# neilcouture/halo2-svd041

Measured on AMD Instinct MI355X. Metric: advice cells/sec (SVD-verify witness gen, N×N) at 1/2/4/8 MI355X, higher is better.
Workload: dtype bn254_fr (u32 limbs; exact multi-modular int8 MFMA GEMM); 1 GPU; svd_verify_witness N=1024 M=1024 PRECISION_BITS=63 LOOKUP_BITS=19, one matrix per GPU; N=1024, M=1024, precision_bits=63, lookup_bits=19, parallelism=replicas x1 (no data-path collective), ranks=1

## Files before the change

### halo2_svd041_amd/csrc/engine.cpp

```cpp
#include <math.h>
#include <stdio.h>
#include <stdlib.h>
#include <string.h>

#include <algorithm>

#include "engine_internal.hpp"
#include "ingest.hpp"
#include "ingest_dev.hpp"
#include "export.hpp"
#include "commit.hpp"

struct BigU {
    Fr v;
};
static BigU big_from_words(const uint64_t w[4]) { return BigU{fr_raw_words(w)}; }
static BigU big_from_u128(unsigned __int128 x) {
    BigU b;
    b.v = fr_zero();
    for (int i = 0; i < 4; ++i) b.v.w[i] = (uint32_t)(x >> (32 * i));
    return b;
}
static int big_bits(const BigU& b) {
    for (int i = 7; i >= 0; --i)
// ... 605 lines not shown
        shard_rows(c, R, &r0, &r1);
        if (R > 1) {
            eb = (uint32_t)(r0 * cw);
            ee = (uint32_t)(r1 * cw);
        }
    }
    if (g_stage_log) {
        uint32_t nmul = 0;
        for (uint32_t i = 0; i < a.nmo; ++i) nmul += a.mo[i].op == MO_MUL;
        const int sid = c->st == c->st_cell ? 1 : c->st == c->st2 ? 2 : c->st == c->st3 ? 3 : 0;
        fprintf(stderr, "stage %-28s elems %8u C %3u L %3u nv %2u nmo %2u muls %u nk %u  s%d\n", tag, ee - eb,
                a.C, a.L, a.nv, a.nmo, nmul, a.nk, sid);
        if (getenv("SVDW_STAGE_LOG")[0] == '2') {
            fprintf(stderr, "  slots");
            for (uint32_t k = 0; k < a.C + a.L; ++k) {
                const SlotOp& o = k < a.C ? a.adv[k] : a.lk[k - a.C];
                fprintf(stderr, " %u:%u:%u", o.src, o.lo, o.nbits);
            }
            fprintf(stderr, "\n");
        }
    }
    if (c->dry || ee <= eb) return;
    a.out_adv = cellp(c, phase, off);
    a.out_lk = a.L ? c->ph[phase].lk + loff : nullptr;
    for (int k = 0; k < kMaxViews; ++k) a.view[k] = f64_view(c, a.view[k]);
    a.e_begin = eb;
    a.e_end = ee;
    a.cols = cols ? cols : 1;
    a.flags = c->opt.stage_flags;
    bool heavy = false;
    for (uint32_t i = 0; i < a.nmo; ++i)
        heavy |= a.mo[i].op == MO_MUL || a.mo[i].op == MO_ISZERO || a.mo[i].op == MO_POWK;
    a.E = heavy ? kStageElems : c->opt.stage_elems;
    while (a.E > 64 && stage_lds_bytes(a.nv ? a.nv : 1, a.E, a.C + a.L) > 65536) a.E -= 64;
    auto magic = [](uint64_t d) -> uint32_t { return d > 1 ? (uint32_t)(((1ull << 32) + d - 1) / d) : 0; };
    a.cdiv_magic = magic(a.C);
    a.ldiv_magic = magic(a.L);
    uint32_t loads = 0;
    for (uint32_t i = 0; i < a.nmo; ++i) loads += a.mo[i].op == MO_LOAD;
    const double bytes = 32.0 * (ee - eb) * ((double)a.C + a.L + loads);
    for (auto& b : c->batches) {
        if (b.st != c->st || !stage_multi_fits(a)) continue;
        auto reads = [&](const svdw_ctx::Pending& q) {
            const char* w0 = reinterpret_cast<const char*>(q.a.out_adv);
            const char* w1 = w0 + sizeof(Fr) * (uint64_t)q.a.e_end * q.a.C;
            for (int k = 0; k < kMaxViews; ++k) {
                const DView& v = a.view[k];
                if (!v.ptr || v.mode == VIEW_DIAGK) continue;
                const int64_t dr = (int64_t)(v.rows ? v.rows - 1 : 0) * v.rs,
                              dc = (int64_t)(v.cols ? v.cols - 1 : 0) * v.cs;
                const int64_t lo = std::min<int64_t>(dr, 0) + std::min<int64_t>(dc, 0),
                              hi = std::max<int64_t>(dr, 0) + std::max<int64_t>(dc, 0) + 1;
                const char* p = reinterpret_cast<const char*>(v.ptr);
                if (p + lo * (int64_t)sizeof(Fr) < w1 && p + hi * (int64_t)sizeof(Fr) > w0) return true;
            }
            return false;
        };
        size_t g = 0;
        for (size_t k = 0; k < b.groups.size(); ++k)
            for (const auto& q : b.groups[k])
                if (reads(q)) g = k + 1;
        if (c->call.stage_front && g == 0) {
            b.groups.insert(b.groups.begin(), std::vector<svdw_ctx::Pending>{});
            b.groups[0].push_back({a, std::string("k_stage:") + tag, bytes});
            b.last = 0;
            return;
        }
// ... 1830 lines not shown
};
template <auto Member>
static void set_opt(svdw_ctx* c, int64_t v) {
    c->opt.*Member = static_cast<std::remove_reference_t<decltype(c->opt.*Member)>>(v);
}
static void set_lanes(svdw_ctx* c, int64_t v) { c->lanes = (int)v; }
static void set_pipeline(svdw_ctx* c, int64_t v) {
    c->opt.pipeline = (int)v;
    if (!v) {
        release_alt(c);
        if (c->lane) release_alt(c->lane);
    }
}
static void set_stage_rot(svdw_ctx* c, int64_t v) {
    c->opt.stage_flags = v ? (c->opt.stage_flags | STAGE_ROT) : (c->opt.stage_flags & ~STAGE_ROT);
}
static const char kStageElemsMsg[] = "stage_elems: a multiple of 16 in [16, 256]";
static void set_stage_elems(svdw_ctx* c, int64_t v) {
    REQUIRE(v % 16 == 0, kStageElemsMsg);
    c->opt.stage_elems = (uint32_t)v;
}
static void set_commit_window_bits(svdw_ctx* c, int64_t v) {
    REQUIRE(v != 1, "commit_window_bits: 0 (the plan) or 2..16");
    c->opt.commit_window_bits = (uint32_t)v;
}
using Opt = svdw_ctx::Options;
static const OptionDef kOptions[] = {
    {"lanes", 1, 2, "lanes: 1 or 2", set_lanes},
    {"pipeline", 0, 1, "pipeline: 0 or 1", set_pipeline},
    {"vm_linear", 0, 1, "vm_linear: 0 or 1", set_opt<&Opt::vm_linear>},
    {"graph", 0, 1, "graph: 0 or 1", set_opt<&Opt::graph_vm>},
    {"gemm_impl", SVDW_GEMM_MFMA, SVDW_GEMM_VALU, "gemm_impl: 0 (mfma) or 1 (valu)", set_opt<&Opt::gemm_impl>},
    {"stage_elems", 16, 256, kStageElemsMsg, set_stage_elems},
    {"prod_cell", -1, 1, "prod_cell: -1, 0 or 1", set_opt<&Opt::prod_cell>},
    {"phase1_overlap", 0, 2, "phase1_overlap: 0, 1 or 2", set_opt<&Opt::phase1_overlap>},
    {"hold_us", 0, 100000, "hold_us: 0..100000", set_opt<&Opt::hold_us>},
    {"rlc_prefix", INT64_MIN, INT64_MAX, "", set_opt<&Opt::rlc_prefix>},
    {"res_f64", INT64_MIN, INT64_MAX, "", set_opt<&Opt::res_f64>},
    {"gemm_crt", 0, 1, "gemm_crt: 0 or 1", set_opt<&Opt::gemm_crt>},
    {"res_wait", -1, 1, "res_wait: -1 (auto), 0 or 1", set_opt<&Opt::res_wait>},
    {"place_trials", 0, 8, "place_trials: 0..8", set_opt<&Opt::place_trials>},
    {"stage_rot", 0, 1, "stage_rot: 0 or 1", set_stage_rot},
    {"gemm_kern", -1, 2, "gemm_kern: -1 (auto), 0, 1 or 2", set_opt<&Opt::gemm_kern>},
    {"stage_batch", INT64_MIN, INT64_MAX, "", set_opt<&Opt::stage_batch>},
    {"f64_views", INT64_MIN, INT64_MAX, "", set_opt<&Opt::f64_views>},
    {"p1_at", -1, 3, "p1_at: -1 (auto), 0, 1, 2 or 3", set_opt<&Opt::p1_at>},
    {"commit_window_bits", 0, kCommitMaxBits, "commit_window_bits: 0 (the plan) or 2..16", set_commit_window_bits},
    {"commit_scratch_mib", 1, 65536, "commit_scratch_mib: 1..65536", set_opt<&Opt::commit_scratch_mib>},
    {"dchk_at", 0, 2, "dchk_at: 0 (cell stream), 1 (st2) or 2 (st3)", set_opt<&Opt::dchk_at>},
    {"gamma_at", -1, 1, "gamma_at: -1 (auto), 0 (cell stream) or 1 (st3)", set_opt<&Opt::gamma_at>},
    {"overlap", INT64_MIN, INT64_MAX, "", set_opt<&Opt::overlap>},
};
static_assert(std::is_nothrow_move_constructible<svdw_ctx>::value && std::is_nothrow_move_assignable<svdw_ctx>::value, "svdw_ctx moves");
static void lane_switch(svdw_ctx* c) {
    if (!c->lane) {
        svdw_ctx* L = new svdw_ctx();
        L->P = c->P;
        L->LB = c->LB;
        L->device = c->device;
        L->dry = false;
        try {
            ctx_init_device(L);
        } catch (...) {
            ctx_release(L);
            throw;
        }
// ... 1516 lines not shown
```

### halo2_svd041_amd/csrc/engine_internal.hpp

```cpp
#pragma once
#include <hip/hip_runtime.h>
#include <stdint.h>

#include <array>
#include <chrono>
#include <functional>
#include <new>
#include <set>
#include <stdexcept>
#include <string>
#include <tuple>
#include <vector>

#include "../../include/svdw.h"
#include "kernels.hpp"

using namespace svdw;

inline thread_local std::string g_err;
struct SvdwError {
    int code;
    std::string msg;
};
[[noreturn]] inline void fail(int code, const std::string& msg) { throw SvdwError{code, msg}; }
// ... 38 lines not shown
inline void fr_store_words(const Fr& x, uint64_t w[4]) {
    for (int i = 0; i < 4; ++i) w[i] = (uint64_t)x.w[2 * i] | ((uint64_t)x.w[2 * i + 1] << 32);
}
inline bool fr_reduced(const Fr& x) {
    Fr t;
    return sub_p(t, x) != 0;
}

struct ProverState {
    DBuf scratch;
    std::vector<char> upload;
    std::vector<Fr> omega;
    uint32_t omega_k = 0;
    DBuf ntt_tab, ntt_tmp;
    uint32_t ntt_k = 0;
    DBuf commit_ws;
    DBuf basis, basis_tmp;
    uint32_t basis_k = 0, basis_ek = 0, basis_unusable = 0;
    Fr basis_shift{};
    std::vector<DBuf*> dbufs() { return {&scratch, &ntt_tab, &ntt_tmp, &basis, &basis_tmp, &commit_ws}; }
};

struct Stream {
    Fr* adv = nullptr;
    uint64_t n = 0, cap = 0;
    Fr* lk = nullptr;
    uint64_t nl = 0, lcap = 0;
};
struct svdw_ctx {
    struct Options {
        int gemm_impl = SVDW_GEMM_MFMA;
        uint32_t stage_flags = STAGE_ALIGN | STAGE_ROT;
        uint32_t stage_elems = kStageElems;
        int gemm_crt = 1;
        int gemm_kern = -1;
        int res_wait = -1;
        int place_trials = 6;
        bool res_f64 = true;
        int phase1_overlap = 1;
        int prod_cell = 1;
        uint32_t hold_us = 0;
        uint32_t commit_window_bits = 0;
        uint32_t commit_scratch_mib = 1024;
        bool rlc_prefix = false;
        int p1_at = -1;
        int dchk_at = 0, gamma_at = -1;
        bool f64_views = true;
        bool overlap = true;
        bool stage_batch = true;
        int graph_vm = 1;
        int vm_linear = 1;
        int pipeline = 1;
        uint32_t shard_rank = 0, shard_world = 1;
        bool prof = false;
        std::string prof_filter;
        bool host_trace = false;
        auto tied() const {
            return std::tie(gemm_impl, stage_flags, stage_elems, gemm_crt, gemm_kern, res_wait, place_trials,
                            res_f64, phase1_overlap, prod_cell, hold_us, rlc_prefix, p1_at, dchk_at, gamma_at,
                            f64_views, overlap, stage_batch, graph_vm, vm_linear, pipeline, shard_rank,
                            shard_world, prof, prof_filter, host_trace);
        }
        bool operator==(const Options& o) const { return tied() == o.tied(); }
    } opt;
    struct PreGemm {
        uint64_t off;
        hipEvent_t ev;
        hipStream_t st;
    };
    struct F64Src { svdw_mat m; const double* x; };
    struct F64Region { uint32_t phase; uint64_t off, n; const double* x; };
    struct Call {
        bool in_pipe = false;
        bool prelaunched = false;
        bool prod_on_cell = false;
        bool gemm_batched = false;
        std::vector<PreGemm> pre;
        hipStream_t pre_wait_st = nullptr;
        hipEvent_t pre_wait_ev = nullptr;
        std::vector<hipEvent_t> gemm_done;
        std::vector<hipEvent_t> wait_before_cs;
        const double* svd_f64[3] = {nullptr, nullptr, nullptr};
        std::vector<F64Region> f64reg;
        std::vector<F64Src> f64src;
        std::function<void(const svdw_svd_payload&)> early_p1;
        bool stage_front = false;
        struct PowsPre {
            bool on = false;
            uint64_t one_off = 0, pows_off = 0;
            uint32_t d = 0;
        } pows_pre;
// ... 171 lines not shown
```

### halo2_svd041_amd/csrc/kernels.hip

```cpp
#include <hip/hip_runtime.h>
#include <hip/hip_ext.h>
#include <type_traits>
#include <string.h>

#include "kernels.hpp"
#include "crt_tables.hpp"
#include "export.hpp"

namespace svdw {

__device__ __forceinline__ double f64_scale(const DView& v) { return ldexp(1.0, (int)v._r0); }
__device__ __forceinline__ Fr view_load(const DView v, const Fr pad, uint32_t i, uint32_t j) {
    if (v.mode == VIEW_DIAG) return (i == j) ? ld_fr(v.ptr) : pad;
    if (v.mode == VIEW_F64) {
        if (i < v.rows && j < v.cols)
            return quantize_fr(reinterpret_cast<const double*>(v.ptr)[(int64_t)i * v.rs + (int64_t)j * v.cs],
                               f64_scale(v));
        return pad;
    }
    if (i < v.rows && j < v.cols) return ld_fr(v.ptr + (int64_t)i * v.rs + (int64_t)j * v.cs);
    return pad;
}
__device__ __forceinline__ uint32_t signed_bits(const Fr& x) {
    Fr half = fr_p();
// ... 467 lines not shown
            }
            default:
                break;
        }
    }
    }

struct StageLds {
    uint32_t* sK;
    uint32_t* sV;
    SlotOp* sAdv;
    SlotOp* sLk;
    MicroOp* sMo;
    DView* sVw;
    uint4* sHM;
    uint32_t* sHD;
};
__device__ __forceinline__ StageLds stage_lds(const StageArgs& a) {
    extern __shared__ __attribute__((aligned(16))) uint32_t smem[];
    StageLds L;
    L.sK = smem;
    L.sV = L.sK + kMaxK * VW;
    const uint32_t E = a.E ? a.E : kStageElems;
    L.sAdv = reinterpret_cast<SlotOp*>(L.sV + E * stage_elem_words(a.nv));
    L.sLk = L.sAdv + kMaxAdv;
    L.sMo = reinterpret_cast<MicroOp*>(L.sLk + kMaxLk);
    L.sVw = reinterpret_cast<DView*>(L.sMo + kMaxMicro);
    static_assert(sizeof(DView) <= 40, "DView grew: recheck stage_lds_bytes");
    const uint32_t hm_off = ((uint32_t)(reinterpret_cast<uint32_t*>(L.sVw + kMaxViews) - smem) + 3u) & ~3u;
    L.sHM = reinterpret_cast<uint4*>(smem + hm_off);
    L.sHD = reinterpret_cast<uint32_t*>(L.sHM + 2 * (a.C + a.L));
    return L;
}
__device__ __forceinline__ void stage_setup(const StageArgs& a, const StageLds& L,
                                            const MicroOp* __restrict__ mo, const SlotOp* __restrict__ adv,
                                            const SlotOp* __restrict__ lk, const Fr* __restrict__ K) {
    const uint32_t tid = threadIdx.x;
    for (uint32_t k = tid; k < a.nk; k += blockDim.x) lds_put(L.sK + k * VW, K[k]);
    for (uint32_t k = tid; k < a.C; k += blockDim.x) L.sAdv[k] = adv[k];
    for (uint32_t k = tid; k < a.L; k += blockDim.x) L.sLk[k] = lk[k];
    for (uint32_t k = tid; k < a.nmo; k += blockDim.x) L.sMo[k] = mo[k];
    if (tid < kMaxViews) L.sVw[tid] = a.view[tid];
    for (uint32_t k = tid; k < 2 * (a.C + a.L); k += blockDim.x) {
        const uint32_t sl = k >> 1;
        make_half(sl < a.C ? adv[sl] : lk[sl - a.C], k & 1, L.sHD + k, L.sHM + k);
    }
}
struct Prefetch {
    Fr v0, v1;
    bool in0, in1;
};
__device__ __forceinline__ Prefetch stage_loads(const StageArgs& a, uint32_t blk) {
    const uint32_t E = a.E ? a.E : kStageElems;
    const uint32_t e0 = a.e_begin + blk * E;
    const uint32_t ne = min(E, a.e_end - e0), e = e0 + threadIdx.x;
    Prefetch f{fr_zero(), fr_zero(), false, false};
    if (threadIdx.x < ne) {
        const uint32_t pi = e / a.cols, pj = e - pi * a.cols;
        const DView& v0 = a.view[0];
        if (v0.ptr && v0.mode == VIEW_STRIDED && pi < v0.rows && pj < v0.cols) {
            f.v0 = ld_fr(v0.ptr + (int64_t)pi * v0.rs + (int64_t)pj * v0.cs);
            f.in0 = true;
        } else if (v0.ptr && v0.mode == VIEW_F64 && pi < v0.rows && pj < v0.cols) {
            f.v0 = quantize_fr(reinterpret_cast<const double*>(v0.ptr)[(int64_t)pi * v0.rs + (int64_t)pj * v0.cs],
                               f64_scale(v0));
            f.in0 = true;
        }
        const DView& v1 = a.view[1];
        if (v1.ptr && v1.mode == VIEW_STRIDED && pi < v1.rows && pj < v1.cols) {
            f.v1 = ld_fr(v1.ptr + (int64_t)pi * v1.rs + (int64_t)pj * v1.cs);
            f.in1 = true;
        } else if (v1.ptr && v1.mode == VIEW_F64 && pi < v1.rows && pj < v1.cols) {
            f.v1 = quantize_fr(reinterpret_cast<const double*>(v1.ptr)[(int64_t)pi * v1.rs + (int64_t)pj * v1.cs],
                               f64_scale(v1));
            f.in1 = true;
        }
    }
    return f;
}
__device__ __forceinline__ void stage_chunk(const StageArgs& a, const StageLds& L, uint32_t blk,
                                            const Prefetch& f) {
    extern __shared__ __attribute__((aligned(16))) uint32_t smem[];
    const uint32_t nv = a.nv, tid = threadIdx.x;
    const uint32_t E = a.E ? a.E : kStageElems;
    const uint32_t e0 = a.e_begin + blk * E;
    const uint32_t ne = min(E, a.e_end - e0), e = e0 + tid;
    if (tid < ne)
        element_program(a, e, L.sV + tid * stage_elem_words(nv), L.sK, L.sMo, L.sVw, f.v0, f.in0, f.v1, f.in1);
    __syncthreads();

    uint4* outA = reinterpret_cast<uint4*>(a.out_adv + (uint64_t)e0 * a.C);
    uint4* outL = a.L ? reinterpret_cast<uint4*>(a.out_lk + (uint64_t)e0 * a.L) : nullptr;
    const uint32_t vb0 = (uint32_t)(L.sV - smem);
    const uint32_t rot = (a.flags & STAGE_ROT) ? blk * 37u : 0u;
    stream_cells_desc<true>(outA, 2 * ne * a.C, L.sHD, L.sHM, a.C, a.cdiv_magic, smem, vb0, nv, rot);
    if (a.L)
        stream_cells_desc<true>(outL, 2 * ne * a.L, L.sHD + 2 * a.C, L.sHM + 2 * a.C, a.L, a.ldiv_magic, smem,
                                vb0, nv, rot);
}

__device__ __forceinline__ void stage_block(const StageArgs& a, const MicroOp* __restrict__ mo,
                                            const SlotOp* __restrict__ adv,
                                            const SlotOp* __restrict__ lk, const Fr* __restrict__ K,
                                            uint32_t blk) {
    const StageLds L = stage_lds(a);
    const Prefetch f = stage_loads(a, blk);
    stage_setup(a, L, mo, adv, lk, K);
    __syncthreads();
    stage_chunk(a, L, blk, f);
}

__global__ __launch_bounds__(256) void k_stage(const StageArgs a) {
    stage_block(a, a.mo, a.adv, a.lk, a.K, blockIdx.x);
}

__device__ __forceinline__ uint32_t multi_prog(const StageMulti& m, uint32_t g) {
    uint32_t p = 0;
    for (uint32_t k = 1; k < m.nprog; ++k) p += g >= m.blk0[k];
    return p;
}
struct Rec {
    const StageArgs* a;
    const MicroOp* mo;
    const SlotOp* adv;
    const SlotOp* lk;
    const Fr* K;
};
__device__ __forceinline__ Rec multi_rec(const StageMulti& m, uint32_t p) {
    const uint8_t* r = m.data + m.off[p];
    Rec q;
    q.a = reinterpret_cast<const StageArgs*>(r);
    q.mo = reinterpret_cast<const MicroOp*>(r + kRecHead);
    q.adv = reinterpret_cast<const SlotOp*>(q.mo + q.a->nmo);
    q.lk = q.adv + q.a->C;
    q.K = reinterpret_cast<const Fr*>(q.lk + q.a->L);
    return q;
}

__global__ __launch_bounds__(256) void k_stage_multi(const StageMulti m) {
    const uint32_t p = multi_prog(m, blockIdx.x);
    const Rec q = multi_rec(m, p);
    stage_block(*q.a, q.mo, q.adv, q.lk, q.K, blockIdx.x - m.blk0[p]);
}
static thread_local hipEvent_t tl_ev0 = nullptr, tl_ev1 = nullptr;
static thread_local bool tl_used = false;
void set_launch_events(hipEvent_t e0, hipEvent_t e1) {
    tl_ev0 = e0;
    tl_ev1 = e1;
    tl_used = false;
}
bool launch_events_used() {
    const bool u = tl_used;
    tl_ev0 = tl_ev1 = nullptr;
    tl_used = false;
    return u;
}
template <class K, class... Args>
static void launch_ev(K kernel, dim3 grid, dim3 block, uint32_t lds, hipStream_t st, Args... args) {
    if (!tl_ev1) {
        hipLaunchKernelGGL(kernel, grid, block, lds, st, args...);
        return;
    }
    hipExtLaunchKernelGGL(kernel, grid, block, lds, st, tl_used ? nullptr : tl_ev0, tl_ev1, 0, args...);
    tl_used = true;
}
hipError_t launch_stage(const StageArgs& a, hipStream_t st) {
    if (a.e_end <= a.e_begin) return hipSuccess;
    const uint32_t n = a.e_end - a.e_begin;
    const uint32_t E = a.E ? a.E : kStageElems;
    if (E > kStageElems) return hipErrorInvalidValue;
    const uint32_t lds = stage_lds_bytes(a.nv ? a.nv : 1, E, a.C + a.L);
    const uint32_t grid = (n + E - 1) / E;
    launch_ev(k_stage, dim3(grid), dim3(256), lds, st, a);
    return hipGetLastError();
}
bool stage_multi_fits(const StageArgs& a) {
    return stage_record_bytes(a.nmo, a.C, a.L, a.nk) <= kMultiBytes && (a.E ? a.E : kStageElems) <= kStageElems;
}
hipError_t launch_stage_multi(const StageArgs* const* progs, int n, hipStream_t st) {
    StageMulti m;
    uint32_t used = 0, blocks = 0, lds = 0;
    m.nprog = 0;
    const StageArgs* single = nullptr;
    auto flush = [&]() -> hipError_t {
        hipError_t e = hipSuccess;
        if (m.nprog == 1) {
            e = launch_stage(*single, st);
        } else if (m.nprog > 1) {
            m.blk0[m.nprog] = blocks;
            launch_ev(k_stage_multi, dim3(blocks), dim3(256), lds, st, m);
            e = hipGetLastError();
        }
        m.nprog = 0;
        used = blocks = lds = 0;
        return e;
    };
    for (int i = 0; i < n; ++i) {
        const StageArgs& a = *progs[i];
        if (a.e_end <= a.e_begin) continue;
        const uint32_t E = a.E ? a.E : kStageElems;
        if (E > kStageElems) return hipErrorInvalidValue;
        const uint32_t rb = stage_record_bytes(a.nmo, a.C, a.L, a.nk);
        if (rb > kMultiBytes) return hipErrorInvalidValue;
        if (m.nprog == (uint32_t)kMaxMulti || used + rb > kMultiBytes) {
            const hipError_t e = flush();
            if (e != hipSuccess) return e;
        }
        uint8_t* r = m.data + used;
        memcpy(r, &a, kRecHead);
        uint8_t* q = r + kRecHead;
        memcpy(q, a.mo, 8 * a.nmo);
        q += 8 * a.nmo;
        memcpy(q, a.adv, 4 * a.C);
        q += 4 * a.C;
        memcpy(q, a.lk, 4 * a.L);
        q += 4 * a.L;
        memcpy(q, a.K, 32 * a.nk);
        m.off[m.nprog] = used;
        m.blk0[m.nprog] = blocks;
        ++m.nprog;
        if (m.nprog == 1) single = &a;
        used += rb;
        blocks += (a.e_end - a.e_begin + E - 1) / E;
        lds = lds > stage_lds_bytes(a.nv ? a.nv : 1, E, a.C + a.L) ? lds : stage_lds_bytes(a.nv ? a.nv : 1, E, a.C + a.L);
    }
    return flush();
}

__global__ __launch_bounds__(256) void k_maxbits(const DView v, uint32_t rows, uint32_t cols,
                                                 unsigned* out) {
    uint64_t n = (uint64_t)rows * cols;
    uint32_t best = 0;
    Fr zero = fr_zero();
    for (uint64_t e = (uint64_t)blockIdx.x * blockDim.x + threadIdx.x; e < n;
         e += (uint64_t)gridDim.x * blockDim.x) {
        uint32_t i = (uint32_t)(e / cols), j = (uint32_t)(e % cols);
        Fr x = view_load(v, zero, i, j);
        best = max(best, signed_bits(x));
    }
    __shared__ uint32_t wmax[4];
#pragma unroll
    for (int off = 32; off > 0; off >>= 1) best = max(best, (uint32_t)__shfl_xor((int)best, off));
    if ((threadIdx.x & 63) == 0) wmax[threadIdx.x >> 6] = best;
    __syncthreads();
    if (threadIdx.x == 0) out[blockIdx.x] = max(max(wmax[0], wmax[1]), max(wmax[2], wmax[3]));
}

hipError_t launch_maxbits(const DView& v, uint32_t rows, uint32_t cols, unsigned* out,
                          hipStream_t st) {
    uint64_t n = (uint64_t)rows * cols;
    if (!n) return hipSuccess;
    unsigned blocks = (unsigned)((n + 255) / 256 < kMaxBitBlocks ? (n + 255) / 256 : kMaxBitBlocks);
    hipLaunchKernelGGL(k_maxbits, dim3(blocks), dim3(256), 0, st, v, rows, cols, out);
    return hipGetLastError();
}

// ... 1640 lines not shown
}
__device__ __forceinline__ U9 u9_add(const U9& a, const U9& b) {
    U9 r;
    uint32_t c = 0;
#pragma unroll
    for (int i = 0; i < 9; ++i) r.w[i] = addc32(a.w[i], b.w[i], c);
    return r;
}
__device__ __forceinline__ U9 u9_sub(const U9& a, const U9& b) {
    U9 r;
    uint32_t br = 0;
#pragma unroll
    for (int i = 0; i < 9; ++i) r.w[i] = subb32(a.w[i], b.w[i], br);
    return r;
}
template <int CTRL, int ROW_MASK>
__device__ __forceinline__ U9 dpp_u9(const U9& v) {
    U9 r;
#pragma unroll
    for (int i = 0; i < 9; ++i)
        r.w[i] = (uint32_t)__builtin_amdgcn_update_dpp(0, (int)v.w[i], CTRL, ROW_MASK, 0xf, true);
    return r;
}
__device__ __forceinline__ U9 wave_scan_u9(U9 s) {
    s = u9_add(s, dpp_u9<0x111, 0xf>(s));
    s = u9_add(s, dpp_u9<0x112, 0xf>(s));
    s = u9_add(s, dpp_u9<0x114, 0xf>(s));
    s = u9_add(s, dpp_u9<0x118, 0xf>(s));
    s = u9_add(s, dpp_u9<0x142, 0xa>(s));
    s = u9_add(s, dpp_u9<0x143, 0xc>(s));
    return s;
}

__device__ __forceinline__ int na_of_bits(uint32_t b) {
    if (b > 192) return 8;
    return b ? (int)((b + 31) / 32) : 1;
}
__device__ __forceinline__ int spec_na(const NaSpec& sp, const unsigned* __restrict__ W) {
    if (sp.wa == -2) return na_of_bits(sp.lk);
    if (sp.wa < 0 || !W) return 8;
    uint32_t b = W[sp.wa];
    if (sp.wb >= 0) b += W[sp.wb] + sp.lk;
    return na_of_bits(b);
}
template <int NA>
__device__ __forceinline__ int batch_na(const ScanBatch& B) {
    if constexpr (NA != 0) {
        return NA;
    } else {
        int na = 1;
#pragma unroll
        for (int q = 0; q < kMaxScanJobs; ++q)
            if ((uint32_t)q < B.njobs) na = max(na, spec_na(B.job[q].spec, B.bitw));
        return na;
    }
}
__device__ __forceinline__ const Fr* tab_slot(const Fr* tab, uint32_t L, int na) {
    return tab + 2ull * (na >= 8 ? kTabSlots - 1 : na - 1) * L;
}
template <int NA>
__device__ __forceinline__ Fr scan_prod(const Fr& a, const Fr* __restrict__ wm,
                                        const Fr* __restrict__ wn, uint32_t j) {
    if constexpr (NA == 8) {
        return mont_mul(a, ld_fr(wm + j));
    } else {
        const bool neg = a.w[7] != 0;
// ... 32 lines not shown
    } else {
        const bool neg = a.w[7] != 0;
        Fr mag = fr_zero(), wv;
        uint32_t br = 0;
#pragma unroll
        for (int q = 0; q < NA; ++q) {
            const uint32_t t = subb32(p_word(q), a.w[q], br);
            mag.w[q] = neg ? t : a.w[q];
        }
#pragma unroll
        for (int q = 0; q < 8; ++q) wv.w[q] = neg ? wnv.w[q] : wmv.w[q];
        return mont_mul_small<NA>(mag, wv);
    }
}
template <int NA>
__device__ __forceinline__ Fr scan_prod_pre(int na, const Fr& a, const Fr& wmv, const Fr& wnv) {
    if constexpr (NA != 0) {
        return scan_prod_v<NA>(a, wmv, wnv);
    } else {
        switch (na) {
        case 1: return scan_prod_v<1>(a, wmv, wnv);
        case 2: return scan_prod_v<2>(a, wmv, wnv);
        case 3: return scan_prod_v<3>(a, wmv, wnv);
        case 4: return scan_prod_v<4>(a, wmv, wnv);
        case 5: return scan_prod_v<5>(a, wmv, wnv);
        case 6: return scan_prod_v<6>(a, wmv, wnv);
        default: return scan_prod_v<8>(a, wmv, wnv);
        }
    }
}

template <int T, int NA>
__global__ __launch_bounds__(256) void k_matvec_scan_dpp(const ScanBatch B) {
    static_assert(256 % T == 0, "T divides the block");
    constexpr uint32_t TPR = 256 / T;
    constexpr uint32_t RS = 6 * T + 1;
    __shared__ __attribute__((aligned(16))) uint4 stage[TPR * RS];
    __shared__ U9 wtot[4], wpre[4];
    __shared__ Fr carry_s;
    ScanJob J = B.job[0];
#pragma unroll
    for (int q = 1; q < kMaxScanJobs; ++q)
        if ((uint32_t)q < B.njobs && blockIdx.x >= B.job[q].blk0) J = B.job[q];
    const DView& A = J.A;
    const uint32_t L = J.L;
    const int na = batch_na<NA>(B);
    const Fr* __restrict__ wc = J.wc;
    const Fr* __restrict__ wm = tab_slot(J.tab, J.tl, na);
    const Fr* __restrict__ wn = wm + J.tl;
    const uint32_t tid = threadIdx.x, lane = tid & 63, wave = tid >> 6;
    const uint32_t lb = blockIdx.x - J.blk0;
    const uint32_t rb = (J.blk0 & 7) ? lb : scan_row(lb, J.rows), r = J.r_begin + rb;
    Fr* rowout = J.out + (uint64_t)rb * (3ull * L + 1);
    const Fr zero = fr_zero();
    Fr eqy = zero;
    if (tid == 0) {
        st_fr(rowout, zero);
        carry_s = zero;
        if (J.eq_out) eqy = ld_fr(J.eq_y + (uint64_t)r * J.eq_ys);
    }
    for (uint32_t c0 = 0; c0 < L; c0 += 256 * T) {
        const uint32_t j0 = c0 + tid * T;
        Fr a[T], w[T], tm[T], tn[T], s[T];
#pragma unroll
        for (int i = 0; i < T; ++i) {
            const uint32_t j = j0 + i;
            const bool in = j < L;
            a[i] = in ? view_load(A, zero, r, j) : zero;
            w[i] = in ? ld_fr(wc + j) : zero;
            tm[i] = in ? ld_fr(wm + j) : zero;
            tn[i] = in && na < 8 ? ld_fr(wn + j) : zero;
        }
#pragma unroll
        for (int i = 0; i < T; ++i) s[i] = j0 + i < L ? scan_prod_pre<NA>(na, a[i], tm[i], tn[i]) : zero;
        U9 loc[T];
        loc[0] = u9_from(s[0]);
#pragma unroll
        for (int i = 1; i < T; ++i) loc[i] = u9_add(loc[i - 1], u9_from(s[i]));
        const U9 tot = wave_scan_u9(loc[T - 1]);
        if (lane == 63) wtot[wave] = tot;
        __syncthreads();
        if (tid == 0) {
            U9 acc = u9_from(carry_s);
#pragma unroll
            for (int w2 = 0; w2 < 4; ++w2) {
                wpre[w2] = acc;
                acc = u9_add(acc, wtot[w2]);
            }
            carry_s = reduce9(acc.w);
        }
        __syncthreads();
        const U9 pre = u9_add(u9_sub(tot, loc[T - 1]), wpre[wave]);
#pragma unroll
        for (int q = 0; q < T; ++q) {
            const uint32_t t0 = c0 + q * 256;
            if (t0 >= L) break;
            if (tid / TPR == (uint32_t)q) {
#pragma unroll
                for (int i = 0; i < T; ++i) {
                    const Fr si = reduce9(u9_add(loc[i], pre).w);
                    uint4* st3 = stage + (tid % TPR) * RS + i * 6;
                    st3[0] = make_uint4(a[i].w[0], a[i].w[1], a[i].w[2], a[i].w[3]);
                    st3[1] = make_uint4(a[i].w[4], a[i].w[5], a[i].w[6], a[i].w[7]);
                    st3[2] = make_uint4(w[i].w[0], w[i].w[1], w[i].w[2], w[i].w[3]);
                    st3[3] = make_uint4(w[i].w[4], w[i].w[5], w[i].w[6], w[i].w[7]);
                    st3[4] = make_uint4(si.w[0], si.w[1], si.w[2], si.w[3]);
                    st3[5] = make_uint4(si.w[4], si.w[5], si.w[6], si.w[7]);
                }
            }
            __syncthreads();
            const uint32_t ncell = 3 * min(256u, L - t0);
            uint4* o = reinterpret_cast<uint4*>(rowout + 1 + 3ull * t0);
            for (uint32_t hc = tid; hc < 2 * ncell; hc += 256) o[hc] = stage[hc + hc / (6 * T)];
            __syncthreads();
        }
    }
    if (J.pc && tid < 1 + kTabSlots) {
        const Fr v = carry_s;
        if (tid == 0) {
            st_fr(J.pc + r, v);
        } else {
            const uint32_t sl = tid - 1;
            const Fr x = mont_mul(v, B.f.f[sl]);
            Fr* base = J.ptab + 2ull * sl * J.plen;
            st_fr(base + r, x);
            if (sl < kTabSlots - 1) st_fr(base + J.plen + r, fr_neg(x));
        }
    }
    if (J.eq_out) {
        if (tid == 0) {
            const Fr x = carry_s, y = eqy;
            const Fr d = fr_sub(x, y), one = fr_from_u64(1);
            const bool z = fr_is_zero(d);
            const Fr zf = z ? one : zero;
            Fr inv = one;
            if (!z) inv = fr_inv(d);
            const Fr cell[12] = {d, y, one, x, zf, d, inv, one, zero, d, zf, zero};
#pragma unroll
            for (int k = 0; k < 12; ++k) {
                stage[2 * k] = make_uint4(cell[k].w[0], cell[k].w[1], cell[k].w[2], cell[k].w[3]);
                stage[2 * k + 1] = make_uint4(cell[k].w[4], cell[k].w[5], cell[k].w[6], cell[k].w[7]);
            }
        }
        __syncthreads();
        if (tid < 24) reinterpret_cast<uint4*>(J.eq_out + 12ull * r)[tid] = stage[tid];
    }
}

template <int NA>
__global__ __launch_bounds__(256) void k_matvec_values(const ScanBatch B) {
    __shared__ U9 part[256];
    ScanJob J = B.job[0];
#pragma unroll
    for (int q = 1; q < kMaxScanJobs; ++q)
        if ((uint32_t)q < B.njobs && blockIdx.x >= B.job[q].blk0) J = B.job[q];
    const DView& A = J.A;
    const uint32_t L = J.L;
    const int na = batch_na<NA>(B);
    const Fr* __restrict__ wm = tab_slot(J.tab, J.tl, na);
    const Fr* __restrict__ wn = wm + J.tl;
    Fr* __restrict__ out = J.out;
    const uint32_t lb = blockIdx.x - J.blk0;
// ... 41 lines not shown
    const double s = round(fabs(x) * scale);
    mag = fr_zero();
    if (s >= 340282366920938463463374607431768211456.0) {
        mag.w[0] = mag.w[1] = mag.w[2] = mag.w[3] = 0xffffffffu;
    } else if (s > 0.0) {
        const uint64_t bits = __double_as_longlong(s);
        const int e = (int)((bits >> 52) & 0x7ff) - 1075;
        const uint64_t mant = (bits & 0xfffffffffffffull) | (1ull << 52);
        const unsigned __int128 v = e >= 0 ? ((unsigned __int128)mant << e) : (unsigned __int128)(mant >> -e);
        mag.w[0] = (uint32_t)v; mag.w[1] = (uint32_t)(v >> 32);
        mag.w[2] = (uint32_t)(v >> 64); mag.w[3] = (uint32_t)(v >> 96);
    }
    neg = signbit(x) && !isnan(x) && s > 0.0;
}
template <int NA>
__device__ __forceinline__ U9 colsum_rows(const double (&x)[kColRows], uint32_t jl0, double scale,
                                          const Fr* sWm, const Fr* sWn) {
    U9 acc = u9_from(fr_zero());
#pragma unroll
    for (int t = 0; t < kColRows; ++t) {
        Fr mag;
        bool neg;
        quantize_mag(x[t], scale, mag, neg);
        const uint32_t jl = jl0 + t;
        Fr s;
        if constexpr (NA == 8) s = mont_mul(neg ? fr_neg(mag) : mag, sWm[jl]);
        else s = mont_mul_small<NA>(mag, neg ? sWn[jl] : sWm[jl]);
        acc = u9_add(acc, u9_from(s));
    }
    return acc;
}
__global__ __launch_bounds__(256) void k_colsum_f64(const ColBatch B, double scale) {
    constexpr uint32_t SR = 8 * kColRows;
    __shared__ Fr sWm[SR], sWn[SR];
    __shared__ U9 sPart[256];
    const ColJob J = B.job[blockIdx.y];
    const uint32_t ncb = (J.C + 31) / 32, cb = blockIdx.x % ncb, sg = blockIdx.x / ncb;
    if (sg * SR >= J.R) return;
    const uint32_t tid = threadIdx.x, col = tid & 31, sub = tid >> 5;
    const uint32_t i = cb * 32 + col, jb = sg * SR, jl0 = sub * kColRows;
    int na = spec_na(J.spec, B.bitw);
    if (na > 4) na = 8;
    const Fr* __restrict__ wm = tab_slot(B.tab, B.tl, na);
    const Fr* __restrict__ wn = wm + B.tl;
    double x[kColRows];
#pragma unroll
    for (int t = 0; t < kColRows; ++t) {
        const uint32_t j = jb + jl0 + t;
        x[t] = i < J.C && j < J.R ? J.x[(uint64_t)j * J.ld + i] : 0.0;
    }
    for (uint32_t k = tid; k < SR; k += 256) {
        const uint32_t j = min(jb + k, J.R - 1);
        sWm[k] = ld_fr(wm + j);
        sWn[k] = na == 8 ? fr_zero() : ld_fr(wn + j);
    }
    __syncthreads();
    U9 acc;
    switch (na) {
    case 1: acc = colsum_rows<1>(x, jl0, scale, sWm, sWn); break;
    case 2: acc = colsum_rows<2>(x, jl0, scale, sWm, sWn); break;
    case 3: acc = colsum_rows<3>(x, jl0, scale, sWm, sWn); break;
    case 4: acc = colsum_rows<4>(x, jl0, scale, sWm, sWn); break;
    default: acc = colsum_rows<8>(x, jl0, scale, sWm, sWn); break;
    }
    sPart[tid] = acc;
    __syncthreads();
    if (sub == 0 && i < J.C) {
#pragma unroll
        for (int k = 1; k < 8; ++k) acc = u9_add(acc, sPart[tid + 32 * k]);
        st_fr(J.part + (uint64_t)sg * J.C + i, reduce9(acc.w));
    }
}
uint32_t colsum_slices(uint32_t R) { return (R + 8 * kColRows - 1) / (8 * kColRows); }
hipError_t launch_colsum_f64(const ColBatch& b, int precision_bits, hipStream_t st) {
    if (!b.njobs || b.njobs > (uint32_t)kMaxColJobs) return hipErrorInvalidValue;
    uint32_t blocks = 0;
    for (uint32_t q = 0; q < b.njobs; ++q) {
        const ColJob& j = b.job[q];
        if (!j.R || j.R > b.tl || j.R > 8192 || j.ld < j.C) return hipErrorInvalidValue;
        blocks = max(blocks, (j.C + 31) / 32 * colsum_slices(j.R));
    }
    if (!blocks) return hipSuccess;
    hipLaunchKernelGGL(k_colsum_f64, dim3(blocks, b.njobs), dim3(256), 0, st, b,
                       (double)(1ull << precision_bits));
    return hipGetLastError();
}
__global__ __launch_bounds__(256) void k_vec_prep_sum(const Fr* __restrict__ part, uint32_t S, uint32_t L,
                                                      Fr* wc, Fr* tab, const ScaleTab f) {
    const uint32_t j = blockIdx.x * blockDim.x + threadIdx.x;
    if (j >= L) return;
    Fr v = fr_zero();
    for (uint32_t s0 = 0; s0 < S; s0 += kColPartBatch) {
        Fr p[kColPartBatch];
#pragma unroll
        for (int s = 0; s < kColPartBatch; ++s)
            p[s] = s0 + s < S ? ld_fr(part + (uint64_t)(s0 + s) * L + j) : fr_zero();
#pragma unroll
        for (int s = 0; s < kColPartBatch; ++s) v = fr_add(v, p[s]);
// ... 90 lines not shown
```

### halo2_svd041_amd/csrc/prog.hpp

```cpp
#pragma once
#include <stddef.h>
#include <stdint.h>

#include "fr.hpp"

namespace svdw {

enum : uint32_t { VIEW_STRIDED = 0, VIEW_DIAG = 1, VIEW_DIAGK = 2, VIEW_F64 = 3 };
struct DView {
    const Fr* ptr;
    int64_t rs, cs;
    uint32_t rows, cols;
    uint32_t mode;
    uint8_t pad_k, diag_k, _r0, _r1;
};

enum : uint8_t {
    MO_LOAD = 1,
    MO_ADDK,
    MO_SUB,
    MO_MUL,
    MO_LIMBSHL,
    MO_FDBL,
    MO_ISZERO,
    MO_POWK,
    MO_SHR,
    MO_ISQRT,
};
struct MicroOp {
    uint8_t op, dst, a, b;
    uint16_t p0, p1;
};

struct SlotOp {
    uint8_t src, lo, nbits, _pad;
};
static constexpr uint8_t KSRC = 0x80;

static constexpr uint32_t STAGE_ALIGN = 256;
static constexpr uint32_t STAGE_ROT = 512;

static constexpr int kMaxViews = 2;
static constexpr int kMaxMicro = 16;
static constexpr int kMaxAdv = 160;
static constexpr int kMaxLk = 48;
static constexpr int kMaxK = 32;
static constexpr int kMaxV = 12;

struct StageArgs {
    Fr* out_adv;
    Fr* out_lk;
    uint32_t e_begin, e_end;
    uint32_t cols;
    uint32_t C, L;
    uint32_t nv, nmo, nk;
    uint32_t flags;
    uint32_t cdiv_magic;
    uint32_t ldiv_magic;
    uint32_t E;
    DView view[kMaxViews];
    MicroOp mo[kMaxMicro];
    SlotOp adv[kMaxAdv];
    SlotOp lk[kMaxLk];
    Fr K[kMaxK];
};
static_assert(sizeof(StageArgs) < 4096, "kernel argument block too large");

static constexpr uint32_t kRecHead = (uint32_t)offsetof(StageArgs, mo);
static_assert(kRecHead % 8 == 0, "record head keeps 8-byte alignment");
constexpr uint32_t stage_record_bytes(uint32_t nmo, uint32_t C, uint32_t L, uint32_t nk) {
    return (kRecHead + 8 * nmo + 4 * (C + L) + 32 * nk + 7) / 8 * 8;
}
static constexpr int kMaxMulti = 16;
static constexpr uint32_t kMultiBytes = 3712;
struct StageMulti {
    uint32_t nprog;
    uint32_t blk0[kMaxMulti + 1];
    uint32_t off[kMaxMulti];
    uint32_t _pad;
    alignas(8) uint8_t data[kMultiBytes];
};
static_assert(sizeof(StageMulti) < 4096, "kernel argument block too large");

static constexpr uint32_t kHalfElem = 0x80000000u;
constexpr uint32_t half_desc(uint32_t off, uint32_t r, bool elem) {
    return off | (r << 16) | (elem ? kHalfElem : 0u);
}
static constexpr uint32_t kStageLdsPad = 64;

constexpr uint32_t stage_elem_words(uint32_t nv) { return nv * 8 + 4; }

constexpr uint32_t stage_lds_bytes(uint32_t nv, uint32_t E, uint32_t CL = kMaxAdv + kMaxLk) {
    return kMaxK * 32 + E * stage_elem_words(nv) * 4 + (kMaxAdv + kMaxLk) * 4 + kMaxMicro * 8 + kMaxViews * 48 +
           CL * 2 * 20 + kStageLdsPad;
}

}
```

Measured before the change: 137.2 billion advice cells/s.

## Process multiple stage chunks per block with software-prefetched view loads

Lets each stage block loop over several element chunks (auto two for large light stages), prefetching the next chunk's view values while computing the current one, and amortizing the per-block table setup. Stage setup is rewritten into single-pass loads before LDS writes. F64 quantization is deferred to use time so the prefetch only issues raw loads. The matvec scan uses a fixed 64 threads per row and colsum aliases its LDS tables with the partials buffer to cut shared-memory use. Fewer blocks may reduce parallelism for mid-size stages.

```diff
diff --git a/halo2_svd041_amd/csrc/engine.cpp b/halo2_svd041_amd/csrc/engine.cpp
--- a/halo2_svd041_amd/csrc/engine.cpp
+++ b/halo2_svd041_amd/csrc/engine.cpp
@@ -661,7 +661,9 @@
     for (uint32_t i = 0; i < a.nmo; ++i)
         heavy |= a.mo[i].op == MO_MUL || a.mo[i].op == MO_ISZERO || a.mo[i].op == MO_POWK;
     a.E = heavy ? kStageElems : c->opt.stage_elems;
+    a.nch = heavy ? 1 : c->opt.stage_chunks;
     while (a.E > 64 && stage_lds_bytes(a.nv ? a.nv : 1, a.E, a.C + a.L) > 65536) a.E -= 64;
+    if (!a.nch) a.nch = (ee - eb + a.E - 1) / a.E >= kStageChunksAutoMin ? 2 : 1;
     auto magic = [](uint64_t d) -> uint32_t { return d > 1 ? (uint32_t)(((1ull << 32) + d - 1) / d) : 0; };
     a.cdiv_magic = magic(a.C);
     a.ldiv_magic = magic(a.L);
@@ -2558,6 +2560,7 @@
     {"graph", 0, 1, "graph: 0 or 1", set_opt<&Opt::graph_vm>},
     {"gemm_impl", SVDW_GEMM_MFMA, SVDW_GEMM_VALU, "gemm_impl: 0 (mfma) or 1 (valu)", set_opt<&Opt::gemm_impl>},
     {"stage_elems", 16, 256, kStageElemsMsg, set_stage_elems},
+    {"stage_chunks", 0, kMaxStageChunks, "stage_chunks: 0 (by stage size) or 1..4", set_opt<&Opt::stage_chunks>},
     {"prod_cell", -1, 1, "prod_cell: -1, 0 or 1", set_opt<&Opt::prod_cell>},
     {"phase1_overlap", 0, 2, "phase1_overlap: 0, 1 or 2", set_opt<&Opt::phase1_overlap>},
     {"hold_us", 0, 100000, "hold_us: 0..100000", set_opt<&Opt::hold_us>},
diff --git a/halo2_svd041_amd/csrc/engine_internal.hpp b/halo2_svd041_amd/csrc/engine_internal.hpp
--- a/halo2_svd041_amd/csrc/engine_internal.hpp
+++ b/halo2_svd041_amd/csrc/engine_internal.hpp
@@ -94,6 +94,7 @@
         int gemm_impl = SVDW_GEMM_MFMA;
         uint32_t stage_flags = STAGE_ALIGN | STAGE_ROT;
         uint32_t stage_elems = kStageElems;
+        uint32_t stage_chunks = 0;
         int gemm_crt = 1;
         int gemm_kern = -1;
         int res_wait = -1;
@@ -118,7 +119,7 @@
         std::string prof_filter;
         bool host_trace = false;
         auto tied() const {
-            return std::tie(gemm_impl, stage_flags, stage_elems, gemm_crt, gemm_kern, res_wait, place_trials,
+            return std::tie(gemm_impl, stage_flags, stage_elems, stage_chunks, gemm_crt, gemm_kern, res_wait, place_trials,
                             res_f64, phase1_overlap, prod_cell, hold_us, rlc_prefix, p1_at, dchk_at, gamma_at,
                             f64_views, overlap, stage_batch, graph_vm, vm_linear, pipeline, shard_rank,
                             shard_world, prof, prof_filter, host_trace);
diff --git a/halo2_svd041_amd/csrc/kernels.hip b/halo2_svd041_amd/csrc/kernels.hip
--- a/halo2_svd041_amd/csrc/kernels.hip
+++ b/halo2_svd041_amd/csrc/kernels.hip
@@ -523,49 +523,77 @@
     L.sHD = reinterpret_cast<uint32_t*>(L.sHM + 2 * (a.C + a.L));
     return L;
 }
+static_assert(kMaxK <= 256 && kMaxAdv <= 256 && kMaxLk <= 256 && kMaxMicro <= 256 &&
+              2 * (kMaxAdv + kMaxLk) <= 512, "stage_setup: one pass per table, two for the halves");
 __device__ __forceinline__ void stage_setup(const StageArgs& a, const StageLds& L,
                                             const MicroOp* __restrict__ mo, const SlotOp* __restrict__ adv,
                                             const SlotOp* __restrict__ lk, const Fr* __restrict__ K) {
-    const uint32_t tid = threadIdx.x;
-    for (uint32_t k = tid; k < a.nk; k += blockDim.x) lds_put(L.sK + k * VW, K[k]);
-    for (uint32_t k = tid; k < a.C; k += blockDim.x) L.sAdv[k] = adv[k];
-    for (uint32_t k = tid; k < a.L; k += blockDim.x) L.sLk[k] = lk[k];
-    for (uint32_t k = tid; k < a.nmo; k += blockDim.x) L.sMo[k] = mo[k];
-    if (tid < kMaxViews) L.sVw[tid] = a.view[tid];
-    for (uint32_t k = tid; k < 2 * (a.C + a.L); k += blockDim.x) {
-        const uint32_t sl = k >> 1;
-        make_half(sl < a.C ? adv[sl] : lk[sl - a.C], k & 1, L.sHD + k, L.sHM + k);
-    }
+    const uint32_t tid = threadIdx.x, nh = 2 * (a.C + a.L);
+    const uint32_t k0 = tid, k1 = tid + 256, s0 = k0 >> 1, s1 = k1 >> 1;
+    Fr kv = fr_zero();
+    SlotOp av = SlotOp{0, 0, 0, 0}, lv = av, h0 = av, h1 = av;
+    MicroOp mv = MicroOp{0, 0, 0, 0, 0, 0};
+    if (tid < a.nk) kv = K[tid];
+    if (tid < a.C) av = adv[tid];
+    if (tid < a.L) lv = lk[tid];
+    if (tid < a.nmo) mv = mo[tid];
+    if (k0 < nh) h0 = s0 < a.C ? adv[s0] : lk[s0 - a.C];
+    if (k1 < nh) h1 = s1 < a.C ? adv[s1] : lk[s1 - a.C];
+    if (tid < a.nk) lds_put(L.sK + tid * VW, kv);
+    if (tid < a.C) L.sAdv[tid] = av;
+    if (tid < a.L) L.sLk[tid] = lv;
+    if (tid < a.nmo) L.sMo[tid] = mv;
+    static_assert(kMaxViews == 2, "stage_setup: the views by constant index (scalar loads)");
+    if (tid == 0) L.sVw[0] = a.view[0];
+    if (tid == 1) L.sVw[1] = a.view[1];
+    if (k0 < nh) make_half(h0, k0 & 1, L.sHD + k0, L.sHM + k0);
+    if (k1 < nh) make_half(h1, k1 & 1, L.sHD + k1, L.sHM + k1);
+}
+__host__ __device__ __forceinline__ uint32_t stage_chunk_count(const StageArgs& a) {
+    const uint32_t E = a.E ? a.E : kStageElems;
+    return (a.e_end - a.e_begin + E - 1) / E;
+}
+__host__ __device__ __forceinline__ uint32_t stage_block_chunks(const StageArgs& a) { return a.nch ? a.nch : 1u; }
+__host__ __device__ __forceinline__ uint32_t stage_block_count(const StageArgs& a) {
+    const uint32_t n = stage_block_chunks(a);
+    return (stage_chunk_count(a) + n - 1) / n;
 }
 struct Prefetch {
     Fr v0, v1;
     bool in0, in1;
 };
-__device__ __forceinline__ Prefetch stage_loads(const StageArgs& a, uint32_t blk) {
+__device__ __forceinline__ void view_prefetch(const DView& v, uint32_t pi, uint32_t pj, Fr& raw, bool& in) {
+    if (!v.ptr || pi >= v.rows || pj >= v.cols) return;
+    const int64_t at = (int64_t)pi * v.rs + (int64_t)pj * v.cs;
+    if (v.mode == VIEW_STRIDED) {
+        raw = ld_fr(v.ptr + at);
+        in = true;
+    } else if (v.mode == VIEW_F64) {
+        const uint64_t bits = (uint64_t)__double_as_longlong(reinterpret_cast<const double*>(v.ptr)[at]);
+        raw.w[0] = (uint32_t)bits;
+        raw.w[1] = (uint32_t)(bits >> 32);
+        in = true;
+    }
+}
+__device__ __forceinline__ Fr prefetch_value(const DView& v, const Fr& raw) {
+    Fr r = raw;
+    if (v.mode == VIEW_F64) {
+        const Fr q = quantize_fr(__longlong_as_double((long long)((uint64_t)raw.w[0] | ((uint64_t)raw.w[1] << 32))),
+                                 f64_scale(v));
+#pragma unroll
+        for (int w = 0; w < 8; ++w) r.w[w] = q.w[w];
+    }
+    return r;
+}
+__device__ __forceinline__ Prefetch stage_loads(const StageArgs& a, uint32_t blk, bool on = true) {
     const uint32_t E = a.E ? a.E : kStageElems;
     const uint32_t e0 = a.e_begin + blk * E;
     const uint32_t ne = min(E, a.e_end - e0), e = e0 + threadIdx.x;
     Prefetch f{fr_zero(), fr_zero(), false, false};
-    if (threadIdx.x < ne) {
+    if (on && threadIdx.x < ne) {
         const uint32_t pi = e / a.cols, pj = e - pi * a.cols;
-        const DView& v0 = a.view[0];
-        if (v0.ptr && v0.mode == VIEW_STRIDED && pi < v0.rows && pj < v0.cols) {
-            f.v0 = ld_fr(v0.ptr + (int64_t)pi * v0.rs + (int64_t)pj * v0.cs);
-            f.in0 = true;
-        } else if (v0.ptr && v0.mode == VIEW_F64 && pi < v0.rows && pj < v0.cols) {
-            f.v0 = quantize_fr(reinterpret_cast<const double*>(v0.ptr)[(int64_t)pi * v0.rs + (int64_t)pj * v0.cs],
-                               f64_scale(v0));
-            f.in0 = true;
-        }
-        const DView& v1 = a.view[1];
-        if (v1.ptr && v1.mode == VIEW_STRIDED && pi < v1.rows && pj < v1.cols) {
-            f.v1 = ld_fr(v1.ptr + (int64_t)pi * v1.rs + (int64_t)pj * v1.cs);
-            f.in1 = true;
-        } else if (v1.ptr && v1.mode == VIEW_F64 && pi < v1.rows && pj < v1.cols) {
-            f.v1 = quantize_fr(reinterpret_cast<const double*>(v1.ptr)[(int64_t)pi * v1.rs + (int64_t)pj * v1.cs],
-                               f64_scale(v1));
-            f.in1 = true;
-        }
+        view_prefetch(a.view[0], pi, pj, f.v0, f.in0);
+        view_prefetch(a.view[1], pi, pj, f.v1, f.in1);
     }
     return f;
 }
@@ -577,7 +605,8 @@
     const uint32_t e0 = a.e_begin + blk * E;
     const uint32_t ne = min(E, a.e_end - e0), e = e0 + tid;
     if (tid < ne)
-        element_program(a, e, L.sV + tid * stage_elem_words(nv), L.sK, L.sMo, L.sVw, f.v0, f.in0, f.v1, f.in1);
+        element_program(a, e, L.sV + tid * stage_elem_words(nv), L.sK, L.sMo, L.sVw, prefetch_value(a.view[0], f.v0),
+                        f.in0, prefetch_value(a.view[1], f.v1), f.in1);
     __syncthreads();
 
     uint4* outA = reinterpret_cast<uint4*>(a.out_adv + (uint64_t)e0 * a.C);
@@ -595,10 +624,18 @@
                                             const SlotOp* __restrict__ lk, const Fr* __restrict__ K,
                                             uint32_t blk) {
     const StageLds L = stage_lds(a);
-    const Prefetch f = stage_loads(a, blk);
+    const uint32_t n = stage_block_chunks(a), c0 = blk * n;
+    const uint32_t c1 = min(c0 + n, stage_chunk_count(a));
+    Prefetch f = stage_loads(a, c0);
     stage_setup(a, L, mo, adv, lk, K);
     __syncthreads();
-    stage_chunk(a, L, blk, f);
+    for (uint32_t ch = c0; ch < c1; ++ch) {
+        const bool more = ch + 1 < c1;
+        const Prefetch g = stage_loads(a, more ? ch + 1 : ch, more);
+        stage_chunk(a, L, ch, f);
+        if (more) __syncthreads();
+        f = g;
+    }
 }
 
 __global__ __launch_bounds__(256) void k_stage(const StageArgs a) {
@@ -657,12 +694,10 @@
 }
 hipError_t launch_stage(const StageArgs& a, hipStream_t st) {
     if (a.e_end <= a.e_begin) return hipSuccess;
-    const uint32_t n = a.e_end - a.e_begin;
     const uint32_t E = a.E ? a.E : kStageElems;
-    if (E > kStageElems) return hipErrorInvalidValue;
+    if (E > kStageElems || a.nch > (uint32_t)kMaxStageChunks) return hipErrorInvalidValue;
     const uint32_t lds = stage_lds_bytes(a.nv ? a.nv : 1, E, a.C + a.L);
-    const uint32_t grid = (n + E - 1) / E;
-    launch_ev(k_stage, dim3(grid), dim3(256), lds, st, a);
+    launch_ev(k_stage, dim3(stage_block_count(a)), dim3(256), lds, st, a);
     return hipGetLastError();
 }
 bool stage_multi_fits(const StageArgs& a) {
@@ -690,7 +725,7 @@
         const StageArgs& a = *progs[i];
         if (a.e_end <= a.e_begin) continue;
         const uint32_t E = a.E ? a.E : kStageElems;
-        if (E > kStageElems) return hipErrorInvalidValue;
+        if (E > kStageElems || a.nch > (uint32_t)kMaxStageChunks) return hipErrorInvalidValue;
         const uint32_t rb = stage_record_bytes(a.nmo, a.C, a.L, a.nk);
         if (rb > kMultiBytes) return hipErrorInvalidValue;
         if (m.nprog == (uint32_t)kMaxMulti || used + rb > kMultiBytes) {
@@ -712,7 +747,7 @@
         ++m.nprog;
         if (m.nprog == 1) single = &a;
         used += rb;
-        blocks += (a.e_end - a.e_begin + E - 1) / E;
+        blocks += stage_block_count(a);
         lds = lds > stage_lds_bytes(a.nv ? a.nv : 1, E, a.C + a.L) ? lds : stage_lds_bytes(a.nv ? a.nv : 1, E, a.C + a.L);
     }
     return flush();
@@ -2419,6 +2454,7 @@
     return s;
 }
 
+static constexpr uint32_t kScanTpr = 64;
 __device__ __forceinline__ int na_of_bits(uint32_t b) {
     if (b > 192) return 8;
     return b ? (int)((b + 31) / 32) : 1;
@@ -2517,8 +2553,8 @@
 
 template <int T, int NA>
 __global__ __launch_bounds__(256) void k_matvec_scan_dpp(const ScanBatch B) {
-    static_assert(256 % T == 0, "T divides the block");
-    constexpr uint32_t TPR = 256 / T;
+    constexpr uint32_t TPR = kScanTpr, NR = 256 / TPR;
+    constexpr uint32_t RT = TPR * T;
     constexpr uint32_t RS = 6 * T + 1;
     __shared__ __attribute__((aligned(16))) uint4 stage[TPR * RS];
     __shared__ U9 wtot[4], wpre[4];
@@ -2577,8 +2613,8 @@
         __syncthreads();
         const U9 pre = u9_add(u9_sub(tot, loc[T - 1]), wpre[wave]);
 #pragma unroll
-        for (int q = 0; q < T; ++q) {
-            const uint32_t t0 = c0 + q * 256;
+        for (int q = 0; q < (int)NR; ++q) {
+            const uint32_t t0 = c0 + q * RT;
             if (t0 >= L) break;
             if (tid / TPR == (uint32_t)q) {
 #pragma unroll
@@ -2594,7 +2630,7 @@
                 }
             }
             __syncthreads();
-            const uint32_t ncell = 3 * min(256u, L - t0);
+            const uint32_t ncell = 3 * min(RT, L - t0);
             uint4* o = reinterpret_cast<uint4*>(rowout + 1 + 3ull * t0);
             for (uint32_t hc = tid; hc < 2 * ncell; hc += 256) o[hc] = stage[hc + hc / (6 * T)];
             __syncthreads();
@@ -2613,6 +2649,7 @@
         }
     }
     if (J.eq_out) {
+        static_assert(TPR * RS >= 24, "the is_equal cells fit the stage");
         if (tid == 0) {
             const Fr x = carry_s, y = eqy;
             const Fr d = fr_sub(x, y), one = fr_from_u64(1);
@@ -2720,8 +2757,11 @@
 }
 __global__ __launch_bounds__(256) void k_colsum_f64(const ColBatch B, double scale) {
     constexpr uint32_t SR = 8 * kColRows;
-    __shared__ Fr sWm[SR], sWn[SR];
-    __shared__ U9 sPart[256];
+    constexpr uint32_t kTabBytes = 2 * SR * sizeof(Fr), kPartBytes = 256 * sizeof(U9);
+    __shared__ __attribute__((aligned(16))) uint8_t sRaw[kTabBytes > kPartBytes ? kTabBytes : kPartBytes];
+    Fr* sWm = reinterpret_cast<Fr*>(sRaw);
+    Fr* sWn = sWm + SR;
+    U9* sPart = reinterpret_cast<U9*>(sRaw);
     const ColJob J = B.job[blockIdx.y];
     const uint32_t ncb = (J.C + 31) / 32, cb = blockIdx.x % ncb, sg = blockIdx.x / ncb;
     if (sg * SR >= J.R) return;
@@ -2751,7 +2791,8 @@
     case 4: acc = colsum_rows<4>(x, jl0, scale, sWm, sWn); break;
     default: acc = colsum_rows<8>(x, jl0, scale, sWm, sWn); break;
     }
-    sPart[tid] = acc;
+    __syncthreads();
+    if (sub) sPart[tid] = acc;
     __syncthreads();
     if (sub == 0 && i < J.C) {
 #pragma unroll
diff --git a/halo2_svd041_amd/csrc/prog.hpp b/halo2_svd041_amd/csrc/prog.hpp
--- a/halo2_svd041_amd/csrc/prog.hpp
+++ b/halo2_svd041_amd/csrc/prog.hpp
@@ -46,6 +46,8 @@
 static constexpr int kMaxLk = 48;
 static constexpr int kMaxK = 32;
 static constexpr int kMaxV = 12;
+static constexpr int kMaxStageChunks = 4;
+static constexpr uint32_t kStageChunksAutoMin = 8192;
 
 struct StageArgs {
     Fr* out_adv;
@@ -58,6 +60,7 @@
     uint32_t cdiv_magic;
     uint32_t ldiv_magic;
     uint32_t E;
+    uint32_t nch;
     DView view[kMaxViews];
     MicroOp mo[kMaxMicro];
     SlotOp adv[kMaxAdv];
@@ -72,7 +75,7 @@
     return (kRecHead + 8 * nmo + 4 * (C + L) + 32 * nk + 7) / 8 * 8;
 }
 static constexpr int kMaxMulti = 16;
-static constexpr uint32_t kMultiBytes = 3712;
+static constexpr uint32_t kMultiBytes = 3840;
 struct StageMulti {
     uint32_t nprog;
     uint32_t blk0[kMaxMulti + 1];
```

Measured after the change: 132.7 billion advice cells/s. 3.3% lower.
